# ha7ilm/csdr

Measured on AMD Instinct MI355X. Metric: complex MS/s in->out, WFM demod chain @2.4 MS/s x N streams, higher is better.
Workload: dtype f32

## Files before the change

csdr_amd/csrc/wfmrx.hip:

```cpp
#include "bank.hpp"
#include "audio_dev.hpp"
#include <math.h>
#include <string.h>

using namespace csdr_amd;

namespace {

constexpr int WF_G = 8;
constexpr int WF_TO = 256;
constexpr int WF_SPAN = 1536;
constexpr int WF_BATCH = 3;
constexpr int WF_RP = WF_SPAN + 4;
constexpr int WF_PAD = 4;

struct WfmrxArgs {
    const float2 *in; size_t in_pitch; int n_in;
    const float2 *last;
    const float *carry; int carry_pitch;
    int held, n_ch;
};

__device__ __forceinline__ float wfmrx_input(const WfmrxArgs &a, const float2 *x, const float *held, int ch, int i)
{
    if (i < 0) return 0.f;
    if (i < a.held) return held[i];
    const int k = i - a.held;
    if (k >= a.n_in) return 0.f;
    const float2 s = x[k], p = k ? x[k - 1] : a.last[ch];
    return fmdemod_quadri(s.x, s.y, p.x, p.y);
}

template <int P>
__global__ __launch_bounds__(256) void k_wfmrx_front(WfmrxArgs a, const int *__restrict__ lo, const float *__restrict__ frac, int n_out, int tile_out,
                                                     const float *__restrict__ denom, float *__restrict__ out, size_t out_pitch)
{
    __shared__ __attribute__((aligned(16))) float rows[WF_G * WF_RP];
    const int tid = threadIdx.x, lane = tid & 63, wv = tid >> 6;
    const int k0 = blockIdx.x * tile_out, kn = min(tile_out, n_out - k0);
    const int c0 = blockIdx.y * WF_G;
    const int first = lo[k0];
    const int s0 = first - ((first - a.held) & 1);
    const int len = min(lo[k0 + kn - 1] + P - s0, WF_SPAN);
    const int nquads = (len + 3) >> 2;
    const bool can = a.n_in >= 6;
    const int k_hi = (a.n_in - 4) & ~1;
    for (int g = wv; g < WF_G; g += 4) {
        const int ch = min(c0 + g, a.n_ch - 1);
        const float2 *x = a.in + (size_t)ch * a.in_pitch;
        const float *held = a.carry + (size_t)ch * a.carry_pitch;
        for (int j0 = 0; 64 * j0 < nquads; j0 += WF_BATCH) {
            float4 U[WF_BATCH], V[WF_BATCH]; float2 Q[WF_BATCH];
            if (can) {
#pragma unroll
                for (int j = 0; j < WF_BATCH; j++) {
                    const int qd = lane + 64 * (j0 + j), k = s0 - a.held + 4 * qd;
                    const int kc = qd < nquads ? min(max(k, 2), k_hi) : 2;
                    Q[j] = x[kc - 1];
                    U[j] = *reinterpret_cast<const float4 *>(x + kc); V[j] = *reinterpret_cast<const float4 *>(x + kc + 2);
                }
            }
#pragma unroll
            for (int j = 0; j < WF_BATCH; j++) {
                const int qd = lane + 64 * (j0 + j), i = s0 + 4 * qd, k = i - a.held;
                if (qd >= nquads) continue;
                float4 d;
                if (k >= 2 && k + 3 < a.n_in) {
                    const float4 u = U[j], v = V[j]; const float2 p = Q[j];
                    d.x = fmdemod_quadri(u.x, u.y, p.x, p.y); d.y = fmdemod_quadri(u.z, u.w, u.x, u.y);
                    d.z = fmdemod_quadri(v.x, v.y, u.z, u.w); d.w = fmdemod_quadri(v.z, v.w, v.x, v.y);
                } else {
                    d.x = wfmrx_input(a, x, held, ch, i); d.y = wfmrx_input(a, x, held, ch, i + 1);
                    d.z = wfmrx_input(a, x, held, ch, i + 2); d.w = wfmrx_input(a, x, held, ch, i + 3);
                }
                *reinterpret_cast<float4 *>(rows + g * WF_RP + 4 * qd) = d;
            }
        }
    }
    __syncthreads();
    if (tid >= kn) return;
    const float fx = frac[k0 + tid];
    const int l = min(max(lo[k0 + tid] - s0, 0), WF_SPAN - P);
    float cf[P];
#pragma unroll
    for (int w = 0; w < P; w++) cf[w] = fracdec_coeff(fx, w, P, -(P / 2) + 1, denom[w]);
#pragma unroll
    for (int g = 0; g < WF_G; g++) {
        if (c0 + g >= a.n_ch) break;
        const float *r = rows + g * WF_RP + l;
        float acc = 0.f;
#pragma unroll
        for (int w = 0; w < P; w++) acc += cf[w] * r[w];
        out[(size_t)(c0 + g) * out_pitch + k0 + tid] = acc;
    }
}

__global__ __launch_bounds__(256) void k_wfmrx_keep(WfmrxArgs a, int from, int rem, float *keep, float2 *__restrict__ last_out)
{
    const int ch = blockIdx.y, j = blockIdx.x * 256 + threadIdx.x;
    const float2 *x = a.in + (size_t)ch * a.in_pitch;
    if (j == 0) last_out[ch] = x[a.n_in - 1];
    if (j >= rem) return;
    const int i = from + j;
    if (i < a.held && keep == a.carry) return;
    keep[(size_t)ch * a.carry_pitch + j] = wfmrx_input(a, x, a.carry + (size_t)ch * a.carry_pitch, ch, i);
}

constexpr int WT_CH = 16, WT_T = 256, WT_RP = WT_T + 1, WT_U = 16;
__device__ __forceinline__ void wfmrx_tail_load(float *buf, const float *__restrict__ in, size_t in_pitch, int c0, int nrows, int t0, int n, int w3, int lane)
{
    for (int r = w3; r < nrows; r += 3) {
        const float *src = in + (size_t)(c0 + r) * in_pitch + t0;
#pragma unroll
        for (int q = 0; q < WT_T / 64; q++) if (t0 + lane + 64 * q < n) buf[r * WT_RP + lane + 64 * q] = src[lane + 64 * q];
    }
}
__device__ __forceinline__ void wfmrx_tail_store(const float *buf, int16_t *__restrict__ out_s16, float *__restrict__ out_f, size_t out_pitch, int c0, int nrows, int t0, int n,
                                                 int w, int nw, int lane)
{
    for (int r = w; r < nrows; r += nw) {
        const size_t o = (size_t)(c0 + r) * out_pitch + t0;
#pragma unroll
        for (int q = 0; q < WT_T / 64; q++) {
            const int t = lane + 64 * q;
            if (t0 + t >= n) continue;
            const float v = buf[r * WT_RP + t];
            if (out_f) out_f[o + t] = v;
            if (out_s16) out_s16[o + t] = (int16_t)f_to_s16(v);
        }
    }
}
__global__ __launch_bounds__(256) void k_wfmrx_tail(const float *__restrict__ in, size_t in_pitch, int n_ch, int n, float alpha, float *__restrict__ state,
                                                    int16_t *__restrict__ out_s16, float *__restrict__ out_f, size_t out_pitch)
{
    __shared__ float tile[3][WT_CH * WT_RP];
    const int tid = threadIdx.x, lane = tid & 63, wv = tid >> 6;
    const int c0 = blockIdx.x * WT_CH, nrows = min(WT_CH, n_ch - c0);
    const float one_minus = 1 - alpha;
    float y = 0.f;
    if (wv == 0 && lane < nrows) { y = state[c0 + lane]; if (y != y) y = 0.f; }
    if (wv) wfmrx_tail_load(tile[0], in, in_pitch, c0, nrows, 0, n, wv - 1, lane);
    __syncthreads();
    const int n_tiles = (n + WT_T - 1) / WT_T;
    for (int t = 0; t < n_tiles; t++) {
        const int t0 = t * WT_T, cols = min(WT_T, n - t0);
        if (wv == 0) {
            if (lane < nrows) {
                float *row = tile[t % 3] + lane * WT_RP;
                int k = 0;
                for (; k + WT_U <= cols; k += WT_U) {
                    float v[WT_U];
#pragma unroll
                    for (int e = 0; e < WT_U; e++) v[e] = row[k + e];
#pragma unroll
                    for (int e = 0; e < WT_U; e++) { y = deemph_wfm_step(alpha, one_minus, v[e], y); v[e] = y; }
#pragma unroll
                    for (int e = 0; e < WT_U; e++) row[k + e] = v[e];
                }
                for (; k < cols; k++) { y = deemph_wfm_step(alpha, one_minus, row[k], y); row[k] = y; }
            }
        } else {
            if (t) wfmrx_tail_store(tile[(t - 1) % 3], out_s16, out_f, out_pitch, c0, nrows, t0 - WT_T, n, wv - 1, 3, lane);
            if (t + 1 < n_tiles) wfmrx_tail_load(tile[(t + 1) % 3], in, in_pitch, c0, nrows, t0 + WT_T, n, wv - 1, lane);
        }
        __syncthreads();
    }
    wfmrx_tail_store(tile[(n_tiles - 1) % 3], out_s16, out_f, out_pitch, c0, nrows, (n_tiles - 1) * WT_T, n, wv, 4, lane);
    if (wv == 0 && lane < nrows) state[c0 + lane] = y;
}

struct WfmrxWalk { long long n_out; float where; long long base; };
WfmrxWalk wfmrx_walk(float rate, int P, int taps, int W, float where, long long total)
{
    WfmrxWalk r{0, where, 0};
    const int xifirst = -(P / 2) + 1;
    while (r.base + W <= total) {
        int hi;
        for (; (hi = (int)ceilf(r.where)) + P + taps < W; r.where += rate) r.n_out++;
        const int processed = (hi - 1) + xifirst;
        r.where -= processed;
        if (processed <= 0) break;
        r.base += processed;
    }
    return r;
}

int wfmrx_check(float rate, int P, int taps, int W)
{
    if (!(rate > 1.0f) || !(rate <= 1e6f)) return fail_msg(-3, "wfmrx: rate should be > 1 (and at most 1e6)");
    if (P < 2 || P > 64 || (P & 1)) return fail_msg(-3, "wfmrx: num_poly_points should be even, 2 .. 64");
    if (taps < 0 || taps > (1 << 16)) return fail_msg(-3, "wfmrx: taps_length should be 0 .. 65536");
    if (W > (1 << 24)) return fail_msg(-3, "wfmrx: window should be at most 2^24");
    if (W < 3 * P / 2 + taps + 1) return fail_msg(-3, "wfmrx: window %d is too short: a window call advances by at least one sample from 3 * num_poly_points / 2 + taps_length + 1 = %d on", W, 3 * P / 2 + taps + 1);
    if (ceilf(rate) > (float)(3 * P / 2 + taps + 1)) return fail_msg(-3, "wfmrx: rate %g is too large for %d points and %d taps: a window call would advance beyond its window (ceil(rate) <= 3 * num_poly_points / 2 + taps_length + 1)", rate, P, taps);
    return 0;
}

}

struct csdr_amd_wfmrx : Bank {
    float rate, tau, alpha; int P, taps_length, W, audio_rate, held, tile_out;
    size_t max_n, d_pitch, a_pitch;
    Owned<csdr_amd_fracdec, csdr_amd_fracdec_destroy> fd;
    DevBuf<cf32> d_last[2]; int lflip;
    DevBuf<float> d_dem;
    DevBuf<float> d_carry[2]; int cflip;
    enum { HELD_BOTH, HELD_DEM, HELD_CARRY } where_held;
    DevBuf<float> d_pre;
    DevBuf<int16_t> d_s16;
    DevBuf<float> d_state;
};

extern "C" {

int csdr_amd_wfmrx_plan(float rate, int num_poly_points, int taps_length, int window, float where, int held, long long n_in, long long *n_out, float *new_where, int *new_held)
{
    const int W = window ? window : 1024;
    if (const int rc = wfmrx_check(rate, num_poly_points, taps_length, W)) return rc;
    if (held < 0 || n_in < 0 || !(where >= 0.f) || !(where <= (float)W)) return fail_msg(-3, "wfmrx: plan needs held >= 0, n_in >= 0 and 0 <= where <= window");
    WfmrxWalk r{0, where, 0};
    if (n_in > 0) r = wfmrx_walk(rate, num_poly_points, taps_length, W, where, held + n_in);
    if (held + n_in - r.base > 0x7fffffffLL) return fail_msg(-3, "wfmrx: plan: the held input exceeds an int");
    if (n_out) *n_out = r.n_out;
    if (new_where) *new_where = r.where;
    if (new_held) *new_held = (int)(held + n_in - r.base);
    return 0;
}

csdr_amd_wfmrx *csdr_amd_wfmrx_create(csdr_amd_ctx *ctx, int n_channels, float rate, int num_poly_points, const float *host_prefilter_taps, int taps_length, int window,
                                      float tau, int audio_rate, size_t max_samples_per_call)
{
    if (bank_create_check("wfmrx", ctx, n_channels, 65535) < 0) return nullptr;
    const int W = window ? window : 1024, nt = host_prefilter_taps ? taps_length : 0;
    if (wfmrx_check(rate, num_poly_points, nt, W) < 0) return nullptr;
    if (!(tau > 0) || audio_rate < 1) { fail_msg(-3, "wfmrx: tau should be > 0 and audio_rate >= 1"); return nullptr; }
    if (max_samples_per_call < 1 || max_samples_per_call > ((size_t)1 << 30)) { fail_msg(-3, "wfmrx: max_samples_per_call should be 1 .. 2^30"); return nullptr; }
    Owned<csdr_amd_wfmrx, csdr_amd_wfmrx_destroy> p(new csdr_amd_wfmrx());
    p->c = ctx; p->n_ch = n_channels; p->rate = rate; p->P = num_poly_points; p->taps_length = nt; p->W = W; p->tau = tau; p->audio_rate = audio_rate;
    p->max_n = max_samples_per_call;
    const float dt = (float)(1.0 / audio_rate);
    p->alpha = dt / (tau + dt);
    p->tile_out = (int)std::min((double)WF_TO, floor((WF_SPAN - num_poly_points - 8) / (double)rate));
    p->fd.reset(csdr_amd_fracdec_create(rate, num_poly_points, host_prefilter_taps, nt));
    if (!p->fd) return nullptr;
    csdr_amd_fracdec_set_cli_bufsize(p->fd.get(), W);
    p->d_pitch = (WF_PAD + (size_t)W + p->max_n + 3) & ~(size_t)3;
    p->a_pitch = ((size_t)csdr_amd_wfmrx_max_output(p.get(), (long long)p->max_n) + 7) & ~(size_t)3;
    hipError_t e = hipSuccess;
    auto alloc = [&](auto &b, size_t bytes) { if (e == hipSuccess) e = dev_alloc(b, bytes); };
    alloc(p->d_last[0], sizeof(cf32) * n_channels); alloc(p->d_last[1], sizeof(cf32) * n_channels);
    alloc(p->d_dem, sizeof(float) * p->d_pitch * n_channels);
    alloc(p->d_carry[0], sizeof(float) * (size_t)W * n_channels); alloc(p->d_carry[1], sizeof(float) * (size_t)W * n_channels);
    alloc(p->d_pre, sizeof(float) * p->a_pitch * n_channels);
    alloc(p->d_s16, sizeof(int16_t) * p->a_pitch * n_channels);
    alloc(p->d_state, sizeof(float) * n_channels);
    if (e != hipSuccess) { fail_msg(-2, "wfmrx: out of device memory"); return nullptr; }
    if (hipMemsetAsync(p->d_pre.get(), 0, sizeof(float) * p->a_pitch * n_channels, ctx->stream) != hipSuccess) { fail_msg(-2, "wfmrx: memset"); return nullptr; }
    if (csdr_amd_wfmrx_reset(p.get()) < 0) return nullptr;
    return p.release();
}

int csdr_amd_wfmrx_reset(csdr_amd_wfmrx *p)
{
    if (!p) return fail_msg(-3, "wfmrx: null object");
    hipStream_t st = p->c->stream;
    p->held = 0; p->lflip = p->cflip = 0; p->where_held = csdr_amd_wfmrx::HELD_BOTH;
    csdr_amd_fracdec_set_where(p->fd.get(), (float)(p->P / 2 - 1));
    CSDR_HIP(hipMemsetAsync(p->d_dem.get(), 0, sizeof(float) * p->d_pitch * p->n_ch, st));
    for (int k = 0; k < 2; k++) {
        CSDR_HIP(hipMemsetAsync(p->d_carry[k].get(), 0, sizeof(float) * (size_t)p->W * p->n_ch, st));
        CSDR_HIP(hipMemsetAsync(p->d_last[k].get(), 0, sizeof(cf32) * p->n_ch, st));
    }
    CSDR_HIP(hipMemsetAsync(p->d_state.get(), 0, sizeof(float) * p->n_ch, st));
    return 0;
}

int csdr_amd_wfmrx_reset_channel(csdr_amd_wfmrx *p, int ch)
{
    if (!p || ch < 0 || ch >= p->n_ch) return fail_msg(-3, "wfmrx: channel out of range");
    hipStream_t st = p->c->stream;
    CSDR_HIP(hipMemsetAsync(p->d_dem.get() + (size_t)ch * p->d_pitch, 0, sizeof(float) * p->d_pitch, st));
    for (int k = 0; k < 2; k++) {
        CSDR_HIP(hipMemsetAsync(p->d_carry[k].get() + (size_t)ch * p->W, 0, sizeof(float) * p->W, st));
        CSDR_HIP(hipMemsetAsync(p->d_last[k].get() + ch, 0, sizeof(cf32), st));
    }
    CSDR_HIP(hipMemsetAsync(p->d_state.get() + ch, 0, sizeof(float), st));
    return 0;
}

void csdr_amd_wfmrx_destroy(csdr_amd_wfmrx *p) { destroy_on_stream(p); }
int csdr_amd_wfmrx_force_generic(csdr_amd_wfmrx *p, int on) { return bank_force_generic(p, "wfmrx", on); }
const char *csdr_amd_wfmrx_kernel_name(const csdr_amd_wfmrx *p) { return bank_kernel_name(p); }
int csdr_amd_wfmrx_held(const csdr_amd_wfmrx *p) { return p ? p->held : -1; }
float csdr_amd_wfmrx_where(const csdr_amd_wfmrx *p) { return p ? csdr_amd_fracdec_get_where(p->fd.get()) : -1.f; }

long long csdr_amd_wfmrx_max_output(const csdr_amd_wfmrx *p, long long n_in)
{
    if (!p || n_in <= 0) return 0;
    return (long long)floor(((double)p->W + (double)n_in) / (double)p->rate) + 2;
}
long long csdr_amd_wfmrx_max_out(const csdr_amd_wfmrx *p, long long n_in) { return csdr_amd_wfmrx_max_output(p, n_in); }

static int wfmrx_move_held(csdr_amd_wfmrx *p, bool to_dem)
{
    if (!p->held) return 0;
    float *carry = p->d_carry[p->cflip].get(), *dem = p->d_dem.get() + WF_PAD;
    const size_t cp = sizeof(float) * p->W, dp = sizeof(float) * p->d_pitch, w = sizeof(float) * p->held;
    if (to_dem) CSDR_HIP(hipMemcpy2DAsync(dem, dp, carry, cp, w, p->n_ch, hipMemcpyDeviceToDevice, p->c->stream));
    else CSDR_HIP(hipMemcpy2DAsync(carry, cp, dem, dp, w, p->n_ch, hipMemcpyDeviceToDevice, p->c->stream));
    return 0;
}

long long csdr_amd_wfmrx_process(csdr_amd_wfmrx *p, const csdr_complexf *in, size_t in_pitch, long long n_in, int16_t *audio_s16, float *audio_f, size_t out_pitch)
{
    if (!p) return fail_msg(-3, "wfmrx: null object");
    if (n_in < 0 || (size_t)n_in > p->max_n) return fail_msg(-3, "wfmrx: n_in should be 0 .. max_samples_per_call (%zu)", p->max_n);
    if (!n_in) return 0;
    if (!in || (in_pitch < (size_t)n_in && p->n_ch > 1)) return fail_msg(-3, "wfmrx: in_pitch below n_in");
    csdr_amd_fracdec *fd = p->fd.get();
    long long n_out64 = 0; int rem = 0; float where_after = 0;
    if (csdr_amd_wfmrx_plan(p->rate, p->P, p->taps_length, p->W, fd->where, p->held, n_in, &n_out64, &where_after, &rem) < 0) return -3;
    const int n_out = (int)n_out64, S = p->n_ch, held = p->held, total = held + (int)n_in, from = total - rem;
    if ((size_t)n_out > out_pitch && S > 1) return fail_msg(-3, "wfmrx: out_pitch %zu smaller than the %d audio samples of this call", out_pitch, n_out);
    if (rem >= p->W || (size_t)n_out > p->a_pitch) return fail_msg(-3, "wfmrx: internal: %d held samples, %d outputs", rem, n_out);
    csdr_amd_ctx *c = p->c; hipStream_t st = c->stream;
    const bool windows = total >= p->W;
    const bool fused = !p->force_generic && !p->taps_length && p->P <= 16 && p->tile_out >= 16 && !((uintptr_t)in & 15) && !(in_pitch & 1);
    if (fused) {
        p->last_kernel = "k_wfmrx_front";
        if (p->where_held == csdr_amd_wfmrx::HELD_DEM) { const int rc = wfmrx_move_held(p, false); if (rc) return rc; }
        WfmrxArgs a;
        a.in = (const float2 *)in; a.in_pitch = in_pitch; a.n_in = (int)n_in; a.last = (const float2 *)p->d_last[p->lflip].get();
        a.carry = p->d_carry[p->cflip].get(); a.carry_pitch = p->W; a.held = held; a.n_ch = S;
        if (windows) {
            if (const int rc = fracdec_plan(c, fd, total)) return rc;
            if (fd->plan_outputs != n_out || fd->plan_processed != from) return fail_msg(-3, "wfmrx: internal: the plans disagree (%d / %d outputs, %d / %d samples)", fd->plan_outputs, n_out, fd->plan_processed, from);
            fracdec_commit(fd);
        }
        if (n_out > 0) {
            const dim3 grid(cdiv(n_out, p->tile_out), cdiv(S, WF_G));
#define WF_FRONT(PV) hipLaunchKernelGGL(k_wfmrx_front<PV>, grid, dim3(256), 0, st, a, (const int *)fd->d_lo.get(), (const float *)fd->d_frac.get(), n_out, p->tile_out, (const float *)fd->d_denom.get(), p->d_pre.get(), p->a_pitch)
            switch (p->P) {
            case 2: WF_FRONT(2); break; case 4: WF_FRONT(4); break; case 6: WF_FRONT(6); break; case 8: WF_FRONT(8); break;
            case 10: WF_FRONT(10); break; case 12: WF_FRONT(12); break; case 14: WF_FRONT(14); break; default: WF_FRONT(16); break;
            }
#undef WF_FRONT
            CSDR_LAUNCH_CHECK();
            hipLaunchKernelGGL(k_wfmrx_tail, dim3(cdiv(S, WT_CH)), dim3(256), 0, st, (const float *)p->d_pre.get(), p->a_pitch, S, n_out, p->alpha, p->d_state.get(), audio_s16, audio_f, out_pitch);
            CSDR_LAUNCH_CHECK();
        }
        float *keep = p->d_carry[from > 0 ? p->cflip ^ 1 : p->cflip].get();
        hipLaunchKernelGGL(k_wfmrx_keep, dim3(std::max(cdiv(rem, 256), 1u), S), dim3(256), 0, st, a, from, rem, keep, (float2 *)p->d_last[p->lflip ^ 1].get());
        CSDR_LAUNCH_CHECK();
        if (from > 0) p->cflip ^= 1;
        p->lflip ^= 1;
        p->where_held = csdr_amd_wfmrx::HELD_CARRY;
    } else {
        p->last_kernel = "k_fracdec";
        if (p->where_held == csdr_amd_wfmrx::HELD_CARRY) { const int rc = wfmrx_move_held(p, true); if (rc) return rc; }
        float *dem = p->d_dem.get() + WF_PAD;
        int rc = csdr_amd_fmdemod_quadri_cf(c, in, dem + held, S, (size_t)n_in, in_pitch, p->d_pitch, p->d_last[p->lflip].get());
        if (rc) return rc;
        p->where_held = csdr_amd_wfmrx::HELD_DEM;
        if (windows) {
            int processed = 0;
            const int got = csdr_amd_fractional_decimator_ff(c, fd, dem, p->d_pre.get(), S, total, p->d_pitch, p->a_pitch, &processed);
            if (got < 0) return got;
            if (got != n_out || processed != from) return fail_msg(-3, "wfmrx: internal: the plans disagree (%d / %d outputs, %d / %d samples)", got, n_out, processed, from);
        }
        if (n_out > 0) {
            const size_t op = std::max(out_pitch, (size_t)n_out);
            rc = csdr_amd_deemphasis_wfm_ff(c, p->d_pre.get(), p->d_pre.get(), S, (size_t)n_out, p->a_pitch, p->a_pitch, p->tau, p->audio_rate, p->d_state.get());
            if (rc) return rc;
            if (audio_f) CSDR_HIP(hipMemcpy2DAsync(audio_f, sizeof(float) * op, p->d_pre.get(), sizeof(float) * p->a_pitch, sizeof(float) * n_out, S, hipMemcpyDeviceToDevice, st));
            if (audio_s16) {
                rc = csdr_amd_convert_f_s16(c, p->d_pre.get(), p->d_s16.get(), p->a_pitch * S);
                if (rc) return rc;
                CSDR_HIP(hipMemcpy2DAsync(audio_s16, sizeof(int16_t) * op, p->d_s16.get(), sizeof(int16_t) * p->a_pitch, sizeof(int16_t) * n_out, S, hipMemcpyDeviceToDevice, st));
            }
        }
        if (from > 0) {
            if (rem) CSDR_HIP(hipMemcpy2DAsync(p->d_carry[p->cflip].get(), sizeof(float) * p->W, dem + from, sizeof(float) * p->d_pitch, sizeof(float) * rem, S, hipMemcpyDeviceToDevice, st));
            p->where_held = csdr_amd_wfmrx::HELD_CARRY;
        }
    }
    p->held = rem;
    return n_out;
}

}
```

Measured before the change: 2.967 million.

## Fuse WFM front and de-emphasis tail into one persistent pipelined kernel

Merges the FM demod plus fractional decimator kernel with the de-emphasis and output kernel. The merged kernel has one persistent 512-thread block per 8-channel group. Inside it, 448 bulk threads prefetch and demodulate the input for the next tile and run the FIR for the current one. One wave runs the serial IIR recurrence on staged tiles while the remaining bulk threads write the outputs. This removes the intermediate global buffer round trip and one launch. In exchange, parallelism collapses to cdiv(S,8) blocks that walk all tiles in sequence, which is risky when the stream count is small.

```diff
diff --git a/csdr_amd/csrc/wfmrx.hip b/csdr_amd/csrc/wfmrx.hip
--- a/csdr_amd/csrc/wfmrx.hip
+++ b/csdr_amd/csrc/wfmrx.hip
@@ -9,8 +9,13 @@
 
 constexpr int WF_G = 8;
 constexpr int WF_TO = 256;
-constexpr int WF_SPAN = 1536;
-constexpr int WF_BATCH = 3;
+constexpr int WF_AHEAD = 2;
+constexpr int WF_NT = 512, WF_NB = WF_NT - 64;
+constexpr int WF_SPAN = 1344;
+constexpr int WF_QROW = WF_SPAN / 4;
+constexpr int WF_NQ = (WF_G * WF_QROW + WF_NB - 1) / WF_NB;
+constexpr int WF_PP = WF_TO + 4;
+constexpr int WF_U = 16;
 constexpr int WF_RP = WF_SPAN + 4;
 constexpr int WF_PAD = 4;
 
@@ -31,68 +36,144 @@
     return fmdemod_quadri(s.x, s.y, p.x, p.y);
 }
 
+struct WfTile { int k0, kn, s0, nquads; };
+static_assert(WF_AHEAD == 2, "k_wfmrx_front: tile s + 1 is demodulated and tile s + 2 asked for in step s");
+static_assert(WF_NQ * WF_NB == WF_G * WF_QROW && WF_SPAN % 4 == 0, "the bulk threads' quads cover the staged rows exactly");
 template <int P>
-__global__ __launch_bounds__(256) void k_wfmrx_front(WfmrxArgs a, const int *__restrict__ lo, const float *__restrict__ frac, int n_out, int tile_out,
-                                                     const float *__restrict__ denom, float *__restrict__ out, size_t out_pitch)
+__device__ __forceinline__ WfTile wf_tile(const WfmrxArgs &a, const int *__restrict__ lo, int n_out, int tile_out, int t, int n_tiles)
+{
+    WfTile r{0, 0, 0, 0};
+    if (t >= n_tiles) return r;
+    r.k0 = t * tile_out; r.kn = min(tile_out, n_out - r.k0);
+    const int first = lo[r.k0];
+    r.s0 = first - ((first - a.held) & 1);
+    r.nquads = (min(lo[r.k0 + r.kn - 1] + P - r.s0, WF_SPAN) + 3) >> 2;
+    return r;
+}
+
+#ifndef WFMRX_DIAG
+#define WFMRX_DIAG 0
+#endif
+
+template <int P>
+__global__ __launch_bounds__(WF_NT) __attribute__((amdgpu_waves_per_eu(4, 4))) void k_wfmrx_front(WfmrxArgs a, const int *__restrict__ lo, const float *__restrict__ frac, int n_out, int tile_out,
+                                                       const float *__restrict__ denom, float alpha, float *__restrict__ state,
+                                                       int16_t *__restrict__ out_s16, float *__restrict__ out_f, size_t out_pitch)
 {
     __shared__ __attribute__((aligned(16))) float rows[WF_G * WF_RP];
-    const int tid = threadIdx.x, lane = tid & 63, wv = tid >> 6;
-    const int k0 = blockIdx.x * tile_out, kn = min(tile_out, n_out - k0);
-    const int c0 = blockIdx.y * WF_G;
-    const int first = lo[k0];
-    const int s0 = first - ((first - a.held) & 1);
-    const int len = min(lo[k0 + kn - 1] + P - s0, WF_SPAN);
-    const int nquads = (len + 3) >> 2;
-    const bool can = a.n_in >= 6;
-    const int k_hi = (a.n_in - 4) & ~1;
-    for (int g = wv; g < WF_G; g += 4) {
-        const int ch = min(c0 + g, a.n_ch - 1);
-        const float2 *x = a.in + (size_t)ch * a.in_pitch;
-        const float *held = a.carry + (size_t)ch * a.carry_pitch;
-        for (int j0 = 0; 64 * j0 < nquads; j0 += WF_BATCH) {
-            float4 U[WF_BATCH], V[WF_BATCH]; float2 Q[WF_BATCH];
-            if (can) {
-#pragma unroll
-                for (int j = 0; j < WF_BATCH; j++) {
-                    const int qd = lane + 64 * (j0 + j), k = s0 - a.held + 4 * qd;
-                    const int kc = qd < nquads ? min(max(k, 2), k_hi) : 2;
-                    Q[j] = x[kc - 1];
-                    U[j] = *reinterpret_cast<const float4 *>(x + kc); V[j] = *reinterpret_cast<const float4 *>(x + kc + 2);
+    __shared__ __attribute__((aligned(16))) float pre[3][WF_G * WF_PP];
+    const int tid = threadIdx.x, b = tid - 64;
+    const bool bulk = tid >= 64;
+    const int c0 = blockIdx.x * WF_G, nrows = min(WF_G, a.n_ch - c0);
+    const int n_tiles = (n_out + tile_out - 1) / tile_out;
+    const float one_minus = 1 - alpha;
+    float4 U[WF_NQ], V[WF_NQ]; float2 Q[WF_NQ];
+    auto demod_fetch = [&](const WfTile &T, const WfTile &N, int b) {
+#pragma unroll
+        for (int j = 0; j < WF_NQ; j++) {
+            const int q = b + WF_NB * j, g = q / WF_QROW, qd = q - g * WF_QROW;
+            const int k = T.s0 - a.held + 4 * qd, kn = N.s0 - a.held + 4 * qd;
+            if (q < WF_G * WF_QROW && qd < T.nquads && k >= 2 && k + 3 < a.n_in) {
+                const float4 u = U[j], v = V[j]; const float2 p = Q[j];
+                float4 d;
+                d.x = fmdemod_quadri(u.x, u.y, p.x, p.y); d.y = fmdemod_quadri(u.z, u.w, u.x, u.y);
+                d.z = fmdemod_quadri(v.x, v.y, u.z, u.w); d.w = fmdemod_quadri(v.z, v.w, v.x, v.y);
+                *reinterpret_cast<float4 *>(rows + g * WF_RP + 4 * qd) = d;
+            }
+            if (q < WF_G * WF_QROW && qd < N.nquads && kn >= 2 && kn + 3 < a.n_in) {
+                const float2 *x = a.in + (size_t)min(c0 + g, a.n_ch - 1) * a.in_pitch + kn;
+                Q[j] = x[-1]; U[j] = *reinterpret_cast<const float4 *>(x); V[j] = *reinterpret_cast<const float4 *>(x + 2);
+            }
+            __builtin_amdgcn_sched_barrier(0);
+        }
+#pragma unroll 1
+        for (int j = 0; j < WF_NQ; j++) {
+            const int q = b + WF_NB * j, g = q / WF_QROW, qd = q - g * WF_QROW, i = T.s0 + 4 * qd, k = i - a.held;
+            if (q >= WF_G * WF_QROW || qd >= T.nquads || (k >= 2 && k + 3 < a.n_in)) continue;
+            const int ch = min(c0 + g, a.n_ch - 1);
+            const float2 *x = a.in + (size_t)ch * a.in_pitch;
+            const float *held = a.carry + (size_t)ch * a.carry_pitch;
+#pragma unroll 1
+            for (int e = 0; e < 4; e++) rows[g * WF_RP + 4 * qd + e] = wfmrx_input(a, x, held, ch, i + e);
+        }
+    };
+    float y = 0.f;
+    auto recur = [&](float *row, int from, int to) {
+        int k = from;
+        if (k + WF_U <= to) {
+            float4 nx[WF_U / 4];
+#pragma unroll
+            for (int e = 0; e < WF_U / 4; e++) nx[e] = reinterpret_cast<const float4 *>(row + k)[e];
+            for (; k + WF_U <= to; k += WF_U) {
+                float v[WF_U];
+#pragma unroll
+                for (int e = 0; e < WF_U / 4; e++) { v[4 * e] = nx[e].x; v[4 * e + 1] = nx[e].y; v[4 * e + 2] = nx[e].z; v[4 * e + 3] = nx[e].w; }
+                if (k + 2 * WF_U <= to) {
+#pragma unroll
+                    for (int e = 0; e < WF_U / 4; e++) nx[e] = reinterpret_cast<const float4 *>(row + k + WF_U)[e];
                 }
-            }
-#pragma unroll
-            for (int j = 0; j < WF_BATCH; j++) {
-                const int qd = lane + 64 * (j0 + j), i = s0 + 4 * qd, k = i - a.held;
-                if (qd >= nquads) continue;
-                float4 d;
-                if (k >= 2 && k + 3 < a.n_in) {
-                    const float4 u = U[j], v = V[j]; const float2 p = Q[j];
-                    d.x = fmdemod_quadri(u.x, u.y, p.x, p.y); d.y = fmdemod_quadri(u.z, u.w, u.x, u.y);
-                    d.z = fmdemod_quadri(v.x, v.y, u.z, u.w); d.w = fmdemod_quadri(v.z, v.w, v.x, v.y);
-                } else {
-                    d.x = wfmrx_input(a, x, held, ch, i); d.y = wfmrx_input(a, x, held, ch, i + 1);
-                    d.z = wfmrx_input(a, x, held, ch, i + 2); d.w = wfmrx_input(a, x, held, ch, i + 3);
+#pragma unroll
+                for (int e = 0; e < WF_U; e++) { y = deemph_wfm_step(alpha, one_minus, v[e], y); v[e] = y; }
+#pragma unroll
+                for (int e = 0; e < WF_U / 4; e++) reinterpret_cast<float4 *>(row + k)[e] = make_float4(v[4 * e], v[4 * e + 1], v[4 * e + 2], v[4 * e + 3]);
+            }
+        }
+        for (; k < to; k++) { y = deemph_wfm_step(alpha, one_minus, row[k], y); row[k] = y; }
+    };
+    const WfTile none{0, 0, 0, 0};
+    WfTile cur = none, nxt = wf_tile<P>(a, lo, n_out, tile_out, 0, n_tiles);
+    float fx = 0.f; int l = 0;
+    if (!bulk && tid < nrows) { y = state[c0 + tid]; if (y != y) y = 0.f; }
+    if (bulk && WFMRX_DIAG != 1) demod_fetch(none, nxt, b);
+    for (int s = -1; s < n_tiles + 2; s++) {
+        const WfTile nn = wf_tile<P>(a, lo, n_out, tile_out, s + 2, n_tiles);
+        const bool rec = WFMRX_DIAG != 2 && !bulk && s >= 1 && s <= n_tiles && tid < nrows;
+        float *row = pre[(s + 2) % 3] + (tid & (WF_G - 1)) * WF_PP;
+        const int cols = min(tile_out, n_out - (s - 1) * tile_out), half = (cols / 2) & ~(WF_U - 1);
+        int bv = b;
+        asm volatile("" : "+v"(bv));
+        float fxn = 0.f; int ln = 0;
+        if (bulk && WFMRX_DIAG != 1) {
+            if (b < nxt.kn) { fxn = frac[nxt.k0 + b]; ln = lo[nxt.k0 + b]; }
+            if (b < WF_TO) {
+                if (b < cur.kn) {
+                    const int li = min(max(l - cur.s0, 0), WF_SPAN - P);
+                    float cf[P];
+#pragma unroll
+                    for (int w = 0; w < P; w++) cf[w] = fracdec_coeff(fx, w, P, -(P / 2) + 1, denom[w]);
+                    float *dst = pre[s % 3] + b;
+#pragma unroll 1
+                    for (int g = 0; g < WF_G; g++) {
+                        if (g >= nrows) break;
+                        const float *r = rows + g * WF_RP + li;
+                        float acc = 0.f;
+#pragma unroll
+                        for (int w = 0; w < P; w++) acc += cf[w] * r[w];
+                        dst[g * WF_PP] = acc;
+                    }
                 }
-                *reinterpret_cast<float4 *>(rows + g * WF_RP + 4 * qd) = d;
-            }
-        }
+            } else if (s >= 2) {
+                const int k0 = (s - 2) * tile_out, kn = min(tile_out, n_out - k0);
+                const float *src = pre[(s - 2) % 3];
+#pragma unroll 4
+                for (int e = b - WF_TO; e < WF_G * WF_TO; e += WF_NB - WF_TO) {
+                    const int r = e / WF_TO, t = e - r * WF_TO;
+                    if (t >= kn || r >= nrows) continue;
+                    const float v = src[r * WF_PP + t];
+                    const size_t o = (size_t)(c0 + r) * out_pitch + k0 + t;
+                    if (out_f) out_f[o] = v;
+                    if (out_s16) out_s16[o] = (int16_t)f_to_s16(v);
+                }
+            }
+        }
+        if (rec) recur(row, 0, half);
+        __syncthreads();
+        if (bulk && WFMRX_DIAG != 1) demod_fetch(nxt, nn, bv);
+        if (rec) recur(row, half, cols);
+        fx = fxn; l = ln; cur = nxt; nxt = nn;
+        __syncthreads();
     }
-    __syncthreads();
-    if (tid >= kn) return;
-    const float fx = frac[k0 + tid];
-    const int l = min(max(lo[k0 + tid] - s0, 0), WF_SPAN - P);
-    float cf[P];
-#pragma unroll
-    for (int w = 0; w < P; w++) cf[w] = fracdec_coeff(fx, w, P, -(P / 2) + 1, denom[w]);
-#pragma unroll
-    for (int g = 0; g < WF_G; g++) {
-        if (c0 + g >= a.n_ch) break;
-        const float *r = rows + g * WF_RP + l;
-        float acc = 0.f;
-#pragma unroll
-        for (int w = 0; w < P; w++) acc += cf[w] * r[w];
-        out[(size_t)(c0 + g) * out_pitch + k0 + tid] = acc;
-    }
+    if (!bulk && tid < nrows) state[c0 + tid] = y;
 }
 
 __global__ __launch_bounds__(256) void k_wfmrx_keep(WfmrxArgs a, int from, int rem, float *keep, float2 *__restrict__ last_out)
@@ -104,69 +185,6 @@
     const int i = from + j;
     if (i < a.held && keep == a.carry) return;
     keep[(size_t)ch * a.carry_pitch + j] = wfmrx_input(a, x, a.carry + (size_t)ch * a.carry_pitch, ch, i);
-}
-
-constexpr int WT_CH = 16, WT_T = 256, WT_RP = WT_T + 1, WT_U = 16;
-__device__ __forceinline__ void wfmrx_tail_load(float *buf, const float *__restrict__ in, size_t in_pitch, int c0, int nrows, int t0, int n, int w3, int lane)
-{
-    for (int r = w3; r < nrows; r += 3) {
-        const float *src = in + (size_t)(c0 + r) * in_pitch + t0;
-#pragma unroll
-        for (int q = 0; q < WT_T / 64; q++) if (t0 + lane + 64 * q < n) buf[r * WT_RP + lane + 64 * q] = src[lane + 64 * q];
-    }
-}
-__device__ __forceinline__ void wfmrx_tail_store(const float *buf, int16_t *__restrict__ out_s16, float *__restrict__ out_f, size_t out_pitch, int c0, int nrows, int t0, int n,
-                                                 int w, int nw, int lane)
-{
-    for (int r = w; r < nrows; r += nw) {
-        const size_t o = (size_t)(c0 + r) * out_pitch + t0;
-#pragma unroll
-        for (int q = 0; q < WT_T / 64; q++) {
-            const int t = lane + 64 * q;
-            if (t0 + t >= n) continue;
-            const float v = buf[r * WT_RP + t];
-            if (out_f) out_f[o + t] = v;
-            if (out_s16) out_s16[o + t] = (int16_t)f_to_s16(v);
-        }
-    }
-}
-__global__ __launch_bounds__(256) void k_wfmrx_tail(const float *__restrict__ in, size_t in_pitch, int n_ch, int n, float alpha, float *__restrict__ state,
-                                                    int16_t *__restrict__ out_s16, float *__restrict__ out_f, size_t out_pitch)
-{
-    __shared__ float tile[3][WT_CH * WT_RP];
-    const int tid = threadIdx.x, lane = tid & 63, wv = tid >> 6;
-    const int c0 = blockIdx.x * WT_CH, nrows = min(WT_CH, n_ch - c0);
-    const float one_minus = 1 - alpha;
-    float y = 0.f;
-    if (wv == 0 && lane < nrows) { y = state[c0 + lane]; if (y != y) y = 0.f; }
-    if (wv) wfmrx_tail_load(tile[0], in, in_pitch, c0, nrows, 0, n, wv - 1, lane);
-    __syncthreads();
-    const int n_tiles = (n + WT_T - 1) / WT_T;
-    for (int t = 0; t < n_tiles; t++) {
-        const int t0 = t * WT_T, cols = min(WT_T, n - t0);
-        if (wv == 0) {
-            if (lane < nrows) {
-                float *row = tile[t % 3] + lane * WT_RP;
-                int k = 0;
-                for (; k + WT_U <= cols; k += WT_U) {
-                    float v[WT_U];
-#pragma unroll
-                    for (int e = 0; e < WT_U; e++) v[e] = row[k + e];
-#pragma unroll
-                    for (int e = 0; e < WT_U; e++) { y = deemph_wfm_step(alpha, one_minus, v[e], y); v[e] = y; }
-#pragma unroll
-                    for (int e = 0; e < WT_U; e++) row[k + e] = v[e];
-                }
-                for (; k < cols; k++) { y = deemph_wfm_step(alpha, one_minus, row[k], y); row[k] = y; }
-            }
-        } else {
-            if (t) wfmrx_tail_store(tile[(t - 1) % 3], out_s16, out_f, out_pitch, c0, nrows, t0 - WT_T, n, wv - 1, 3, lane);
-            if (t + 1 < n_tiles) wfmrx_tail_load(tile[(t + 1) % 3], in, in_pitch, c0, nrows, t0 + WT_T, n, wv - 1, lane);
-        }
-        __syncthreads();
-    }
-    wfmrx_tail_store(tile[(n_tiles - 1) % 3], out_s16, out_f, out_pitch, c0, nrows, (n_tiles - 1) * WT_T, n, wv, 4, lane);
-    if (wv == 0 && lane < nrows) state[c0 + lane] = y;
 }
 
 struct WfmrxWalk { long long n_out; float where; long long base; };
@@ -338,15 +356,13 @@
             fracdec_commit(fd);
         }
         if (n_out > 0) {
-            const dim3 grid(cdiv(n_out, p->tile_out), cdiv(S, WF_G));
-#define WF_FRONT(PV) hipLaunchKernelGGL(k_wfmrx_front<PV>, grid, dim3(256), 0, st, a, (const int *)fd->d_lo.get(), (const float *)fd->d_frac.get(), n_out, p->tile_out, (const float *)fd->d_denom.get(), p->d_pre.get(), p->a_pitch)
+            const dim3 grid(cdiv(S, WF_G));
+#define WF_FRONT(PV) hipLaunchKernelGGL(k_wfmrx_front<PV>, grid, dim3(WF_NT), 0, st, a, (const int *)fd->d_lo.get(), (const float *)fd->d_frac.get(), n_out, p->tile_out, (const float *)fd->d_denom.get(), p->alpha, p->d_state.get(), audio_s16, audio_f, out_pitch)
             switch (p->P) {
             case 2: WF_FRONT(2); break; case 4: WF_FRONT(4); break; case 6: WF_FRONT(6); break; case 8: WF_FRONT(8); break;
             case 10: WF_FRONT(10); break; case 12: WF_FRONT(12); break; case 14: WF_FRONT(14); break; default: WF_FRONT(16); break;
             }
 #undef WF_FRONT
-            CSDR_LAUNCH_CHECK();
-            hipLaunchKernelGGL(k_wfmrx_tail, dim3(cdiv(S, WT_CH)), dim3(256), 0, st, (const float *)p->d_pre.get(), p->a_pitch, S, n_out, p->alpha, p->d_state.get(), audio_s16, audio_f, out_pitch);
             CSDR_LAUNCH_CHECK();
         }
         float *keep = p->d_carry[from > 0 ? p->cflip ^ 1 : p->cflip].get();
```

Result: no change. 2.957 million (-0.3%).
